# nrlugg/fenix

Hardware: NVIDIA B200
Metric: knn_qps (higher is better)
Workload: dtype f32

## Files before the change

### fenix_b200/csrc/fenix_knn.cu

```cuda
#include <cuda.h>
#include <cuda_runtime.h>
#include <nvtx3/nvToolsExt.h>

#include <dlfcn.h>
#include <unistd.h>

#include <algorithm>
#include <atomic>
#include <chrono>
#include <cmath>
#include <condition_variable>
#include <cstdarg>
#include <cstdio>
#include <cstdlib>
#include <cstring>
#include <memory>
#include <mutex>
#include <new>
#include <string>
#include <thread>
#include <unordered_map>
#include <vector>

#include "../../include/fenix_knn.h"
// ... 115 lines not shown
  fx::TcCorpus tc;
  struct GraphEntry {
    int64_t n_q = 0; int metric = 0, k = 0, precision = 0;
    int state = 0;
    cudaGraphExec_t exec = nullptr;
    void* ptrs[7] = {nullptr, nullptr, nullptr, nullptr, nullptr, nullptr, nullptr};
    uint64_t knob_epoch = 0;
    int path = 0, variant = 0, launches = 0, operand = 0;
  };
  std::vector<GraphEntry> graphs;
  int* d_inv = nullptr; long long* d_cell_off = nullptr;
  std::vector<long long> h_cell_off;
  int64_t n_inv = 0, n_cells = 0;
};

static int bind(fx_ctx* ctx) {
  FX_CUDA(cudaSetDevice(ctx->device));
  return FX_OK;
}

struct HandleState { int users = 0; bool doomed = false; };
static std::mutex g_reg_mu;
static std::condition_variable g_reg_cv;
static std::unordered_map<const fx_corpus*, HandleState> g_live;

struct Lease {
  const fx_corpus* c;
  bool ok = false;
  explicit Lease(const fx_corpus* c_) : c(c_) {
    if (!c) return;
// ... 576 lines not shown
    s.certify = precision == FX_PREC_FP32; s.out_rows = d_out_rows; s.out_dist = d_out_dist;
    s.stream = ctx->stream; s.ev_k0 = ctx->ev_k0; s.ev_k1 = ctx->ev_k1; s.ev_flags = ev_flags; s.dbg = nullptr; s.tau_fixed = nullptr;
    const bool have_i8 = int8_wanted(c, metric, k, precision) && ensure_i8_shadow(c);
    const bool want_bf16 = precision == FX_PREC_BF16 || (precision == FX_PREC_FP32 && !ctx->tc.knobs.fp32_filter_tf32);
    const bool have_shadow = !have_i8 && want_bf16 && ((metric == 1 && ensure_norm_shadow(c)) || ensure_plain_shadow(c));
    const int kind = have_i8 ? 2 : (have_shadow ? 1 : 0);
    if (precision == FX_PREC_BF16 && !have_shadow)
      return fail(FX_ESTATE, "fx_search: FX_PREC_BF16 needs a bf16 shadow (none could be built: FENIX_BF16_SHADOW=0, a tiny shard, or no HBM left)");
    FX_TRY(configure_filter(c, metric, kind, d_mask, &s));
    run->L = fx::tc_prepare(&ctx->tc, s);
    FX_TRY(ctx->d_tc.ensure(run->L.scratch_bytes));
    std::string err;
    int launched = 0, variant = 0;
    if (!fx::tc_search(&ctx->tc, &c->tc, s, run->L, ctx->d_tc.p, &launched, &err, &variant)) return fail(FX_ECUDA, "fx_search: %s", err.c_str());
    run->tc = true; run->path = kind == 0 ? 1 : 2; run->operand = kind;
    c->stats.last_variant = variant;
    ctx->launches += launched; c->stats.kernel_launches += launched;
    if (s.certify) FX_CUDA(cudaMemcpyAsync(ctx->h_word, fx::tc_flag_count(ctx->d_tc.p), sizeof(int), cudaMemcpyDeviceToHost, ctx->stream));
  } else {
    FX_CUDA(cudaEventRecordWithFlags(ctx->ev_k0, ctx->stream, ev_flags));
    FX_TRY(run_exact_scan(c, d_q, int(n_q), nullptr, int(n_q), metric, k, d_mask, d_out_rows, d_out_dist));
    FX_CUDA(cudaEventRecordWithFlags(ctx->ev_k1, ctx->stream, ev_flags));
  }
  if (!spin) FX_CUDA(cudaEventRecordWithFlags(ctx->ev_stop, ctx->stream, ev_flags));
  return FX_OK;
}

static int search_settle(fx_corpus* c, SearchRun* run, bool* changed) {
  fx_ctx* ctx = c->ctx;
  *changed = false;
  if (!run->tc || !run->s.certify || ctx->h_word[0] == 0) return FX_OK;
// ... 176 lines not shown
  ctx->capturing = false;
  cudaGraph_t graph = nullptr;
  const cudaError_t ee = cudaStreamEndCapture(ctx->stream, &graph);
  if (!ok || ee != cudaSuccess || !graph || !run->tc) {
    cudaGetLastError();
    if (graph) cudaGraphDestroy(graph);
    g->state = -1;
    return false;
  }
  cudaGraphExec_t exec = nullptr;
  if (cudaGraphInstantiate(&exec, graph, 0) != cudaSuccess) { cudaGetLastError(); cudaGraphDestroy(graph); g->state = -1; return false; }
  cudaGraphDestroy(graph);
  g->exec = exec; g->state = 1; g->knob_epoch = ctx->knob_epoch;
  const void* now[7] = {ctx->d_q.p, ctx->d_rows.p, ctx->d_dist.p, ctx->d_tc.p, ctx->h_q.p, ctx->h_rows.p, ctx->h_dist.p};
  for (int i = 0; i < 7; ++i) g->ptrs[i] = const_cast<void*>(now[i]);
  g->path = run->path; g->operand = run->operand; g->variant = c->stats.last_variant; g->launches = int(c->stats.kernel_launches - launches0);
  c->stats.kernel_launches = launches0;
  return true;
}

extern "C" int fx_search(fx_corpus* c, const float* queries, int64_t n_q, int32_t metric, int32_t k,
                         int32_t precision, const uint8_t* row_mask, int64_t* out_rows, float* out_dist) {
  FX_LEASE(c, "fx_search");
  NvtxRange nvtx("fenix:search");
  FX_TRY(check_search_args(c, queries, n_q, metric, k, precision, out_rows, out_dist));
  if (n_q == 0) return FX_OK;
  fx_ctx* ctx = c->ctx;
  std::lock_guard<std::mutex> lock(ctx->mu);
  FX_TRY(bind(ctx));
  const size_t q_bytes = size_t(n_q) * c->dim * sizeof(float);
  const size_t r_bytes = size_t(n_q) * k * sizeof(int64_t), d_bytes = size_t(n_q) * k * sizeof(float);
// ... 55 lines not shown
    if (g->state == 1 && !graph_buffers_match(ctx, *g)) {
      cudaGraphExecDestroy(g->exec); g->exec = nullptr; g->state = 0;
    }
    bool launched = false;
    SearchRun run;
    if (g->state >= 0) {
      FX_TRY(ctx->h_q.ensure(q_bytes));
      FX_TRY(ctx->h_rows.ensure(r_bytes));
      FX_TRY(ctx->h_dist.ensure(d_bytes));
    }
    if (g->state == 1) {
      std::memcpy(ctx->h_q.p, queries, q_bytes);
      ctx->h_word[0] = 0;
      FX_CUDA(cudaGraphLaunch(g->exec, ctx->stream));
      run.tc = true; run.path = g->path; run.operand = g->operand; run.n_q = n_q;
      c->stats.last_variant = g->variant;
      ctx->launches += g->launches; c->stats.kernel_launches += g->launches;
      launched = true;
    } else if (g->state == 2) {
      std::memcpy(ctx->h_q.p, queries, q_bytes);
      if (graph_capture(c, g, n_q, metric, k, precision, q_bytes, r_bytes, d_bytes, &run)) {
        ctx->h_word[0] = 0;
        FX_CUDA(cudaGraphLaunch(g->exec, ctx->stream));
        ctx->launches += g->launches; c->stats.kernel_launches += g->launches;
        launched = true;
      }
    } else if (g->state == 0) {
      g->state = 2;
    }
    if (launched) {
      FX_CUDA(cudaStreamSynchronize(ctx->stream));
// ... 607 lines not shown
```

### fenix_b200/csrc/tc_filter.cuh

```cuda
#pragma once
#include <cuda.h>
#include <cuda_bf16.h>
#include <cuda_runtime.h>

#include <cstdlib>
#include <string>

#include "common.cuh"

namespace fx {

constexpr int TC_BM = 128;
constexpr int TC_BN = 256;
constexpr int TC_BK = 32;
constexpr int TC_UMMA_K = 8;
constexpr int TC_STAGES = 4;
constexpr int TC_ACC_STAGES = 2;
constexpr int TC_SPLIT = 2;
#ifndef FENIX_EPI_UNROLL
#define FENIX_EPI_UNROLL 2
#endif
constexpr int TC_EPI_UNROLL = FENIX_EPI_UNROLL;
constexpr int TC_EPI_WARPS = 4 * TC_SPLIT;
constexpr int TC_THREADS = 32 * (4 + TC_EPI_WARPS);
constexpr int TC_EPI_FIRST_WARP = 4;
constexpr int TC_HALF_COLS = TC_BN / TC_SPLIT;
constexpr int TC_SLOTS = TC_SPLIT * TC_BM;
constexpr int TC_CW = 32;
constexpr uint32_t TC_A_BYTES = TC_BM * TC_BK * 4;
constexpr uint32_t TC_B_BYTES = TC_BN * TC_BK * 4;
constexpr uint32_t TC_STAGE_BYTES = TC_A_BYTES + TC_B_BYTES;
constexpr uint32_t TC_NORM_BYTES = TC_BN * 4;
constexpr uint32_t TC_SMEM_BYTES = 1024  + TC_STAGES * TC_STAGE_BYTES +
                                   TC_ACC_STAGES * TC_NORM_BYTES + 512 ;
constexpr int TC2_STAGES = 6;
constexpr uint32_t TC2_B_BYTES = TC_B_BYTES / 2;
constexpr uint32_t TC2_STAGE_BYTES = TC_A_BYTES + TC2_B_BYTES;
constexpr uint32_t TC2_SMEM_BYTES = 1024  + TC2_STAGES * TC2_STAGE_BYTES +
                                    TC_ACC_STAGES * TC_NORM_BYTES + 512 ;
constexpr size_t TC_HDR_BYTES = 256;
constexpr int TC_MAX_WAVES = 4;
constexpr uint32_t ORD_NEG_INF = 0x007fffffu;

constexpr int TC_AUG_COLS = 4;
struct ShadowGeom {
  int n_kb_data;
  int aug_col;
  bool aug_separate;
  int pitch_q;
};
inline ShadowGeom shadow_geom(int dim) {
  ShadowGeom g;
  g.n_kb_data = (dim + 63) / 64;
  const int used = dim - 64 * (g.n_kb_data - 1);
// ... 37 lines not shown
  int pair = -1;
  int errcol = -1;
  int fp32_filter_tf32 = 0;
  int no_refine = 0;
  int no_norm_shadow = 0;
  int debug_bf16 = 0;
  int graph = 1;
  int debug_tiers = 0;
  int direct = 1;
  int direct_mb = 256;
  int direct_spin = 1;
  int direct_qreg = 0;
  int merge_rank_min = 0;
  int debug_direct = 0;
  int int8 = -1;
};
inline bool tc_set_knob(TcKnobs* k, const char* name, const char* value) {
  const std::string n(name ? name : "");
  const TcKnobs d{};
  auto as_int = [&](int dflt) { return value ? std::atoi(value) : dflt; };
  auto as_flag = [&]() { return (value && std::atoi(value) != 0) ? 1 : 0; };
  auto as_dbl = [&]() { return value ? std::atof(value) : 0.0; };
  if (n == "FENIX_TC_KP") k->kp = as_int(d.kp);
  else if (n == "FENIX_TC_FULLK") k->fullk = as_flag();
  else if (n == "FENIX_TC_NO_RQ") k->no_rq = as_flag();
  else if (n == "FENIX_TC_SLICES") k->slices = as_int(d.slices);
  else if (n == "FENIX_TC_MAX_WAVES") k->max_waves = as_int(d.max_waves);
  else if (n == "FENIX_TC_ORDER") k->order = as_int(d.order);
  else if (n == "FENIX_TC_KP_LIST") k->kp_list = as_int(d.kp_list);
  else if (n == "FENIX_TC_PRE_WIDE") k->pre_wide = as_int(d.pre_wide);
// ... 8 lines not shown
  else if (n == "FENIX_TC_PAIR") k->pair = as_int(d.pair);
  else if (n == "FENIX_TC_ERRCOL") k->errcol = as_int(d.errcol);
  else if (n == "FENIX_FP32_FILTER_TF32") k->fp32_filter_tf32 = as_flag();
  else if (n == "FENIX_NO_REFINE") k->no_refine = as_flag();
  else if (n == "FENIX_NO_NORM_SHADOW") k->no_norm_shadow = as_flag();
  else if (n == "FENIX_DEBUG_BF16") k->debug_bf16 = as_flag();
  else if (n == "FENIX_DEBUG_TIERS") k->debug_tiers = as_flag();
  else if (n == "FENIX_GRAPH") k->graph = as_int(d.graph);
  else if (n == "FENIX_DIRECT") k->direct = as_int(d.direct);
  else if (n == "FENIX_DIRECT_MAX_MB") k->direct_mb = as_int(d.direct_mb);
  else if (n == "FENIX_DEBUG_DIRECT") k->debug_direct = as_flag();
  else if (n == "FENIX_DIRECT_SPIN") k->direct_spin = as_int(d.direct_spin);
  else if (n == "FENIX_DIRECT_QREG") k->direct_qreg = as_int(d.direct_qreg);
  else if (n == "FENIX_MERGE_RANK_MIN") k->merge_rank_min = as_int(d.merge_rank_min);
  else if (n == "FENIX_INT8") k->int8 = as_int(d.int8);
  else return false;
  return true;
}
inline void tc_knobs_from_env(TcKnobs* k) {
  static const char* const names[] = {
      "FENIX_TC_KP", "FENIX_TC_FULLK", "FENIX_TC_NO_RQ", "FENIX_TC_SLICES", "FENIX_TC_MAX_WAVES", "FENIX_TC_ORDER", "FENIX_TC_KP_LIST",
      "FENIX_TC_PRE_WIDE", "FENIX_TC_PRE", "FENIX_TC_PRE_SMALL", "FENIX_TC_PRE_SAFETY", "FENIX_TC_PRE_M", "FENIX_TC_PF", "FENIX_RQ_STAGES",
      "FENIX_FIN_THREADS", "FENIX_TC_WARM", "FENIX_TC_PAIR", "FENIX_TC_ERRCOL", "FENIX_FP32_FILTER_TF32", "FENIX_NO_REFINE",
      "FENIX_NO_NORM_SHADOW", "FENIX_DEBUG_BF16", "FENIX_DEBUG_TIERS", "FENIX_GRAPH", "FENIX_DIRECT", "FENIX_DIRECT_MAX_MB", "FENIX_DEBUG_DIRECT", "FENIX_DIRECT_SPIN", "FENIX_DIRECT_QREG", "FENIX_MERGE_RANK_MIN", "FENIX_INT8"};
  for (const char* name : names) {
    if (const char* v = std::getenv(name)) tc_set_knob(k, name, v);
  }
}

struct TcState {
  int sm_count = 0;
  void* encode = nullptr;
  TcKnobs knobs;
};
struct TcCorpus {
  CUtensorMap map_x;
  CUtensorMap map_xb;
  CUtensorMap map_xn;
  CUtensorMap map_xb_h, map_xn_h;
// ... 529 lines not shown
    uint32_t v_ord = (p.cap == 1024) ? warp_select_compact<32>(b, c_src, p.kp, new_cnt)
                                     : warp_select_compact<16>(b, c_src, p.kp, new_cnt);
    if (int(lane) == src) {
      wn = uint32_t(new_cnt);
      tau = fmaxf(tau, ord2f(v_ord));
      atomicMax(p.tau_g + q, v_ord);
      wn_trig = epi_trigger(p, active, tau);
    }
  }
}

template <int METRIC, int KIND, int MODE, int PAIR>
__global__ void __launch_bounds__(TC_THREADS, 1)
knn_tc_filter_kernel(const __grid_constant__ CUtensorMap map_q, const __grid_constant__ CUtensorMap map_x, TcParams p) {
  static_assert(!PAIR || KIND >= 1, "CTA pairs stream a shadow");
  constexpr int STAGES = PAIR ? TC2_STAGES : TC_STAGES;
  constexpr uint32_t B_BYTES = PAIR ? TC2_B_BYTES : TC_B_BYTES;
  constexpr uint32_t STAGE_BYTES = TC_A_BYTES + B_BYTES;
  extern __shared__ unsigned char smem_raw[];
  unsigned char* smem = smem_raw + ((1024u - (smem_u32(smem_raw) & 1023u)) & 1023u);
  unsigned char* tiles = smem;
  float* norm_smem = reinterpret_cast<float*>(smem + STAGES * STAGE_BYTES);
  uint64_t* bars = reinterpret_cast<uint64_t*>(smem + STAGES * STAGE_BYTES + TC_ACC_STAGES * TC_NORM_BYTES);
  uint64_t* full_bar = bars;
  uint64_t* empty_bar = bars + STAGES;
  uint64_t* tmem_full = bars + 2 * STAGES;
  uint64_t* tmem_empty = tmem_full + TC_ACC_STAGES;
  uint64_t* norm_full = tmem_empty + TC_ACC_STAGES;
  uint64_t* norm_empty = norm_full + TC_ACC_STAGES;
  uint32_t* tmem_ptr = reinterpret_cast<uint32_t*>(norm_empty + TC_ACC_STAGES);

  const int warp = threadIdx.x >> 5;
  const uint32_t lane = lane_id();
  const uint32_t rank = PAIR ? cluster_ctarank() : 0u;
  const int cid = PAIR ? int(blockIdx.x >> 1) : int(blockIdx.x);
  const int n_workers = PAIR ? int(gridDim.x >> 1) : int(gridDim.x);

  if (warp == 0 && lane == 0) {
    prefetch_tmap(&map_q);
    prefetch_tmap(&map_x);
    for (int i = 0; i < STAGES; ++i) { mbar_init(&full_bar[i], 1); mbar_init(&empty_bar[i], 1); }
    for (int i = 0; i < TC_ACC_STAGES; ++i) {
      mbar_init(&tmem_full[i], 1);
      mbar_init(&tmem_empty[i], PAIR ? 2 * TC_EPI_WARPS : TC_EPI_WARPS);
      mbar_init(&norm_full[i], 1);
      mbar_init(&norm_empty[i], TC_EPI_WARPS);
    }
    fence_barrier_init();
  }
  if (warp == 2) { if (PAIR) tmem_alloc_pair(tmem_ptr, 512); else tmem_alloc(tmem_ptr, 512); }
  tc_fence_before();
  __syncthreads();
  if (PAIR) cluster_sync_all();
  tc_fence_after();
  const uint32_t tmem_base = *tmem_ptr;

  const int n_qp = (p.n_qt + 1) >> 1;
  const int n_units = PAIR ? p.n_slices * n_qp : p.n_slices * p.n_qt;
  const int n_rows_i = int(p.n_rows);
  auto decode = [&](int u, int& qt, int& slice, int& cu) {
    if (PAIR) { const int qp = u % n_qp; slice = u / n_qp; qt = 2 * qp + int(rank); cu = slice * (2 * n_qp) + qt; }
    else { qt = p.qt_major ? u / p.n_slices : u % p.n_qt; slice = p.qt_major ? u % p.n_slices : u / p.n_qt; cu = u; }
  };

  if (warp == 0) {
    if (lane == 0) {
      int stage = 0; uint32_t phase = 0;
      int acc = 0; uint32_t acc_phase = 0;
      const uint32_t full_leader = PAIR ? mapa_u32(smem_u32(full_bar), 0) : 0u;
      for (int u = cid; u < n_units; u += n_workers) {
        int qt, slice, cu; decode(u, qt, slice, cu);
        const int t0 = slice * p.tiles_per_slice, t1 = min(p.n_vtiles, t0 + p.tiles_per_slice);
        for (int tv = t0; tv < t1; ++tv) {
          const int t = tv * p.tile_stride;
          if (METRIC != 2) {
            mbar_wait_backoff(PAIR ? &norm_empty[acc] : &tmem_empty[acc], acc_phase ^ 1, p.sleep_ns);
            mbar_expect_tx(&norm_full[acc], TC_NORM_BYTES);
            const float* src = (METRIC == 0 ? p.hx : p.rx) + size_t(t) * TC_BN;
            bulk_load_1d(norm_smem + acc * TC_BN, src, TC_NORM_BYTES, &norm_full[acc]);
          }
          for (int kb = 0; kb < p.n_kblocks; ++kb) {
            mbar_wait_backoff(&empty_bar[stage], phase ^ 1, p.sleep_ns);
            unsigned char* a_dst = tiles + stage * STAGE_BYTES;
            constexpr int kElemsPerBlock = KIND == 0 ? TC_BK : (KIND == 1 ? 2 * TC_BK : 4 * TC_BK);
            const int line = kb < p.n_kb_data ? (t * p.n_kb_data + kb) * TC_BN : p.aug_line0 + t * TC_BN;
            if (PAIR) {
              if (rank == 0) mbar_expect_tx(&full_bar[stage], 2 * STAGE_BYTES);
              const uint32_t bar = full_leader + uint32_t(stage) * 8u;
              tma_load_2d_pair(&map_q, bar, a_dst, kb * kElemsPerBlock, qt * TC_BM);
              tma_load_2d_pair(&map_x, bar, a_dst + TC_A_BYTES, 0, line + int(rank) * (TC_BN / 2));
            } else {
              mbar_expect_tx(&full_bar[stage], STAGE_BYTES);
              tma_load_2d(&map_q, &full_bar[stage], a_dst, kb * kElemsPerBlock, qt * TC_BM);
              if (KIND == 0) tma_load_2d(&map_x, &full_bar[stage], a_dst + TC_A_BYTES, kb * kElemsPerBlock, t * TC_BN);
              else {
                tma_load_2d(&map_x, &full_bar[stage], a_dst + TC_A_BYTES, 0, line);
#ifndef FENIX_NO_PFCODE
                if (p.pf_tiles > 0 && tv + p.pf_tiles < t1) {
                  const int tp = (tv + p.pf_tiles) * p.tile_stride;
                  const int64_t linep = kb < p.n_kb_data ? (int64_t(tp) * p.n_kb_data + kb) * TC_BN : int64_t(p.aug_line0) + int64_t(tp) * TC_BN;
                  prefetch_l2(p.xb + linep * 128, TC_B_BYTES);
                }
#endif
              }
            }
            if (++stage == STAGES) { stage = 0; phase ^= 1; }
          }
          if (++acc == TC_ACC_STAGES) { acc = 0; acc_phase ^= 1; }
        }
      }
    }
  } else if (warp == 1 && rank == 0) {
    {
      constexpr uint32_t idesc = KIND == 0 ? make_idesc_tf32(TC_BM, TC_BN)
                                           : KIND == 1 ? make_idesc_bf16(PAIR ? 2 * TC_BM : TC_BM, TC_BN)
                                                       : make_idesc_i8(PAIR ? 2 * TC_BM : TC_BM, TC_BN);
      const uint32_t tmem_u = __shfl_sync(0xffffffffu, tmem_base, 0);
      const uint64_t desc0 = make_smem_desc(0);
      const uint32_t tiles_lo = smem_u32(tiles) >> 4;
      const int n_kb = p.n_kblocks, n_kb_data = p.n_kb_data, nk_last = p.nk_last;
      int stage = 0; uint32_t phase = 0;
      int acc = 0; uint32_t acc_phase = 0;
      for (int u = cid; u < n_units; u += n_workers) {
        int qt, slice, cu; decode(u, qt, slice, cu);
        const int t0 = slice * p.tiles_per_slice, t1 = min(p.n_vtiles, t0 + p.tiles_per_slice);
        for (int t = t0; t < t1; ++t) {
          mbar_wait_backoff(&tmem_empty[acc], acc_phase ^ 1, p.sleep_ns >> 1);
          const uint32_t d_tmem = tmem_u + uint32_t(acc * TC_BN);
          for (int kb = 0; kb < n_kb; ++kb) {
            mbar_wait(&full_bar[stage], phase);
            tc_fence_after();
            const uint64_t a_desc = desc0 | uint64_t(tiles_lo + uint32_t(stage) * (STAGE_BYTES >> 4));
            const uint64_t b_desc = a_desc + (TC_A_BYTES >> 4);
            const int nk = kb < n_kb_data - 1 ? TC_BK / TC_UMMA_K : (kb == n_kb_data - 1 ? nk_last : 1);
            if (elect_one()) {
              if (PAIR && KIND == 2) {
                umma_i8_pair(d_tmem, a_desc, b_desc, idesc, kb != 0 ? 1u : 0u);
                if (nk > 1) umma_i8_pair(d_tmem, a_desc + 2, b_desc + 2, idesc, 1u);
                if (nk > 2) umma_i8_pair(d_tmem, a_desc + 4, b_desc + 4, idesc, 1u);
                if (nk > 3) umma_i8_pair(d_tmem, a_desc + 6, b_desc + 6, idesc, 1u);
                umma_commit_pair(&empty_bar[stage]);
                if (kb == n_kb - 1) umma_commit_pair(&tmem_full[acc]);
              } else if (PAIR) {
                umma_bf16_pair(d_tmem, a_desc, b_desc, idesc, kb != 0 ? 1u : 0u);
                if (nk > 1) umma_bf16_pair(d_tmem, a_desc + 2, b_desc + 2, idesc, 1u);
                if (nk > 2) umma_bf16_pair(d_tmem, a_desc + 4, b_desc + 4, idesc, 1u);
                if (nk > 3) umma_bf16_pair(d_tmem, a_desc + 6, b_desc + 6, idesc, 1u);
                umma_commit_pair(&empty_bar[stage]);
// ... 8 lines not shown
                  umma_bf16(d_tmem, a_desc, b_desc, idesc, kb != 0 ? 1u : 0u);
                  if (nk > 1) umma_bf16(d_tmem, a_desc + 2, b_desc + 2, idesc, 1u);
                  if (nk > 2) umma_bf16(d_tmem, a_desc + 4, b_desc + 4, idesc, 1u);
                  if (nk > 3) umma_bf16(d_tmem, a_desc + 6, b_desc + 6, idesc, 1u);
                } else {
                  umma_i8(d_tmem, a_desc, b_desc, idesc, kb != 0 ? 1u : 0u);
                  if (nk > 1) umma_i8(d_tmem, a_desc + 2, b_desc + 2, idesc, 1u);
                  if (nk > 2) umma_i8(d_tmem, a_desc + 4, b_desc + 4, idesc, 1u);
                  if (nk > 3) umma_i8(d_tmem, a_desc + 6, b_desc + 6, idesc, 1u);
                }
                umma_commit(&empty_bar[stage]);
                if (kb == n_kb - 1) umma_commit(&tmem_full[acc]);
              }
            }
            __syncwarp();
            if (++stage == STAGES) { stage = 0; phase ^= 1; }
          }
          if (++acc == TC_ACC_STAGES) { acc = 0; acc_phase ^= 1; }
        }
      }
    }
  } else if (warp >= TC_EPI_FIRST_WARP) {
    const int e = warp - TC_EPI_FIRST_WARP;
    const int lane_grp = warp & 3;
    const int half = e >> 2;
    const int row_in_tile = lane_grp * 32 + int(lane);
    const int slot = half * TC_BM + row_in_tile;
    const uint32_t t_lane = tmem_base + (uint32_t(lane_grp * 32) << 16) + uint32_t(half * TC_HALF_COLS);
    const uint32_t tmem_empty_leader = PAIR ? mapa_u32(smem_u32(tmem_empty), 0) : 0u;
    int acc = 0; uint32_t acc_phase = 0;

    for (int u = cid; u < n_units; u += n_workers) {
      int qt, slice, cu; decode(u, qt, slice, cu);
// ... 20 lines not shown
        float2 ts = make_float2(1.f, 0.f);
        if (KIND == 2) ts = __ldg(p.i8_tile + t);
        mbar_wait(&tmem_full[acc], acc_phase);
        if (METRIC != 2) mbar_wait(&norm_full[acc], acc_phase);
        tc_fence_after();
        const int col0 = t * TC_BN + half * TC_HALF_COLS;
        const int ncols = min(TC_HALF_COLS, n_rows_i - col0);
        const float* nrm = norm_smem + acc * TC_BN + half * TC_HALF_COLS;
        float* dbg_row = nullptr;
        if (MODE == 1) { if (u == 0 && tv == t0) dbg_row = p.dbg + (int(lane) * 4 + lane_grp) * TC_BN + half * TC_HALF_COLS; }
        float* pre_out = nullptr;
        if (MODE == 2) { if (active) pre_out = p.pre_max + size_t(q) * p.pre_pitch + (tv * TC_SPLIT + half); }
        if (KIND == 2) {
          const double ss = double(ts.x) * double(qs.x);
          const double ae = fma(double(qs.y), double(ts.y), double(qs.z)) + 0x1p-48;
          epi_tile_i8<METRIC, MODE, PAIR>(t_lane + uint32_t(acc * TC_BN), any_active ? ncols : 0, nrm, col0, tau,
                                          i8_threshold(tau, ss, ae), 1.0 / ss, ae, buf, wn, &tmem_empty[acc],
                                          tmem_empty_leader + uint32_t(acc) * 8u, &norm_empty[acc], lane, dbg_row, pre_out);
        } else {
          epi_tile<METRIC, MODE, PAIR>(t_lane + uint32_t(acc * TC_BN), any_active ? ncols : 0, nrm, col0, tau, buf, wn,
                                       &tmem_empty[acc], tmem_empty_leader + uint32_t(acc) * 8u, &norm_empty[acc], lane, dbg_row, pre_out);
        }
        if (++acc == TC_ACC_STAGES) { acc = 0; acc_phase ^= 1; }
        if (MODE != 2) epi_tighten(p, active, q, buf, wn, wn_trig, tau, lane);
      }

      if (MODE != 2) p.wcnt[size_t(cu) * TC_SLOTS + slot] = active ? int(wn) : 0;
    }
  }

  tc_fence_before();
  __syncthreads();
  if (PAIR) cluster_sync_all();
  if (warp == 2) {
    tc_fence_after();
    if (PAIR) tmem_dealloc_pair(tmem_base, 512); else tmem_dealloc(tmem_base, 512);
// ... 766 lines not shown
    if (a == cudaSuccess) a = cudaFuncSetAttribute(kernel, cudaFuncAttributeMaxDynamicSharedMemorySize, int(bytes));
  };
  attr(knn_tc_filter_kernel<0, 0, 0, 0>, TC_SMEM_BYTES); attr(knn_tc_filter_kernel<1, 0, 0, 0>, TC_SMEM_BYTES);
  attr(knn_tc_filter_kernel<2, 0, 0, 0>, TC_SMEM_BYTES); attr(knn_tc_filter_kernel<0, 1, 0, 0>, TC_SMEM_BYTES);
  attr(knn_tc_filter_kernel<1, 1, 0, 0>, TC_SMEM_BYTES); attr(knn_tc_filter_kernel<2, 1, 0, 0>, TC_SMEM_BYTES);
  attr(knn_tc_filter_kernel<0, 1, 2, 0>, TC_SMEM_BYTES); attr(knn_tc_filter_kernel<1, 1, 2, 0>, TC_SMEM_BYTES);
  attr(knn_tc_filter_kernel<2, 1, 2, 0>, TC_SMEM_BYTES);
  attr(knn_tc_filter_kernel<0, 1, 0, 1>, TC2_SMEM_BYTES); attr(knn_tc_filter_kernel<1, 1, 0, 1>, TC2_SMEM_BYTES);
  attr(knn_tc_filter_kernel<2, 1, 0, 1>, TC2_SMEM_BYTES);
  attr(knn_tc_filter_kernel<0, 1, 2, 1>, TC2_SMEM_BYTES); attr(knn_tc_filter_kernel<1, 1, 2, 1>, TC2_SMEM_BYTES);
  attr(knn_tc_filter_kernel<2, 1, 2, 1>, TC2_SMEM_BYTES);
  attr(knn_tc_filter_kernel<0, 2, 0, 0>, TC_SMEM_BYTES); attr(knn_tc_filter_kernel<2, 2, 0, 0>, TC_SMEM_BYTES);
  attr(knn_tc_filter_kernel<2, 2, 2, 0>, TC_SMEM_BYTES);
  attr(knn_tc_filter_kernel<0, 2, 0, 1>, TC2_SMEM_BYTES); attr(knn_tc_filter_kernel<2, 2, 0, 1>, TC2_SMEM_BYTES);
  attr(knn_tc_filter_kernel<2, 2, 2, 1>, TC2_SMEM_BYTES);
  if (a == cudaSuccess) a = cudaFuncSetAttribute(knn_rq_filter_kernel<0, 0>, cudaFuncAttributeMaxDynamicSharedMemorySize, RQ_SMEM_MAX);
  if (a == cudaSuccess) a = cudaFuncSetAttribute(knn_rq_filter_kernel<0, 2>, cudaFuncAttributeMaxDynamicSharedMemorySize, RQ_SMEM_MAX);
  if (a == cudaSuccess) a = cudaFuncSetAttribute(knn_rq_filter_kernel<2, 2>, cudaFuncAttributeMaxDynamicSharedMemorySize, RQ_SMEM_MAX);
  if (a == cudaSuccess) a = cudaFuncSetAttribute(knn_rq_filter_kernel<2, 0>, cudaFuncAttributeMaxDynamicSharedMemorySize, RQ_SMEM_MAX);
  if (a == cudaSuccess) a = cudaFuncSetAttribute(knn_tc_finish_kernel, cudaFuncAttributeMaxDynamicSharedMemorySize, 64 * 1024);
  if (a != cudaSuccess) { *err = std::string("cudaFuncSetAttribute(tc kernels) failed: ") + cudaGetErrorString(a); return false; }
  return true;
}

inline bool tc_bind_shadow(const TcState* st, CUtensorMap* map, CUtensorMap* map_half, const void* Xb, int64_t n_rows,
                           int blocks_per_tile, std::string* err, int esize = 2) {
  const uint64_t lines = uint64_t((n_rows + TC_BN - 1) / TC_BN) * uint64_t(blocks_per_tile) * TC_BN;
  if (lines >= (uint64_t(1) << 31)) { *err = "shard too large for a tiled shadow (32-bit TMA coordinates)"; return false; }
  const uint32_t line = 128 / esize;
  if (!tc_encode_2d(st, map_half, Xb, line, lines, line, line, TC_BN / 2, err, esize)) return false;
// ... 26 lines not shown
  (void)n_q;
  if (!st->encode || !tc->ok) return false;
  if (dim > 8192) return false;
  if (k > 320) return false;
  if (n_rows < 4096 || n_rows < 8 * int64_t(k)) return false;
  if (n_rows > int64_t(0x7fffff00)) return false;
  return true;
}

struct TcPlan {
  int n_qt, n_tiles, n_slices, tiles_per_slice, grid, units, kp, cap, n_kblocks, n_kb_data, nk_last, aug_line0, aug_col;
  int n_vtiles, tile_stride;
  int qt_major;
  int rq;
  int pair;
  int n_qt_lists;
  int n_qp;
  int kp_list;
  int kb_bf16;
  size_t off_qp, off_qb, off_tau, off_flags, off_qerr, off_wcnt, off_wbuf, off_pre, total;
  int n_rec, pre_pitch;
};

inline TcPlan tc_plan(const TcState* st, const TcSearch& s) {
  TcPlan pl{};
  pl.n_qt = (s.n_q + TC_BM - 1) / TC_BM;
  pl.n_tiles = int((s.n_rows + TC_BN - 1) / TC_BN);
  pl.kp = s.tau_fixed ? 1024 : tc_kp(s.k, s.certify, s.kind);
  const bool pre = s.sample_stride > 1;
  if (pre) pl.kp = 32;
// ... 10 lines not shown
    pl.nk_last = (s.dim - I8_KB * (pl.n_kb_data - 1) + 31) / 32;
    pl.n_kblocks = pl.n_kb_data;
  } else {
    const ShadowGeom g = shadow_geom(s.dim);
    pl.n_kb_data = g.n_kb_data;
    const int used = s.dim - 64 * (g.n_kb_data - 1) + ((s.aug && !g.aug_separate) ? TC_AUG_COLS : 0);
    pl.nk_last = (used + 15) / 16;
    pl.n_kblocks = g.n_kb_data + ((s.aug && g.aug_separate) ? 1 : 0);
    pl.aug_line0 = pl.n_tiles * g.n_kb_data * TC_BN;
    pl.aug_col = g.aug_col;
  }
  if (kn.fullk) pl.nk_last = TC_BK / TC_UMMA_K;
  pl.kb_bf16 = s.kind == 2 ? (s.dim + 63) / 64 : pl.n_kblocks;
  pl.rq = (s.kind == 1 && pl.n_kblocks <= RQ_MAX_KB && pl.n_qt >= 2 && s.epi != 1 && s.dbg == nullptr && !kn.no_rq) ? 1 : 0;
  pl.n_qp = (pl.n_qt + 1) / 2;
  pl.pair = (!pl.rq && s.kind >= 1 && pl.n_qt >= 2 && s.dbg == nullptr && (kn.pair == 1 || (kn.pair < 0 && pl.kb_bf16 >= 7))) ? 1 : 0;
  pl.n_qt_lists = pl.pair ? 2 * pl.n_qp : pl.n_qt;
  const int n_tiles_full = pl.rq ? int((s.n_rows + RQ_BN - 1) / RQ_BN) : pl.n_tiles;
  pl.tile_stride = pre ? s.sample_stride : 1;
  const int n_tiles_u = (n_tiles_full + pl.tile_stride - 1) / pl.tile_stride;
  pl.n_vtiles = n_tiles_u;
  const int n_qu = (pl.rq || pl.pair) ? pl.n_qp : pl.n_qt;
  const int sms = pl.pair ? st->sm_count / 2 : st->sm_count;
  const int min_tiles = pre ? 4 : std::max(4, (8 * pl.kp + TC_BN - 1) / TC_BN) * (pl.rq ? 2 : 1);
  const int max_waves = kn.max_waves > 0 ? kn.max_waves : TC_MAX_WAVES;
  const int s_cap = std::max(1, (max_waves * sms) / n_qu);
  const int s_max = std::max(1, std::min(n_tiles_u / min_tiles, s_cap));
  double best = -1.0; int best_s = 1;
  for (int sl = 1; sl <= s_max; ++sl) {
    int tps = (n_tiles_u + sl - 1) / sl;
    int eff_s = (n_tiles_u + tps - 1) / tps;
// ... 160 lines not shown
    le = cudaLaunchKernelEx(&cfg, kernel, map_q, map_b, p);
  };
  const bool dbg = s.dbg != nullptr;
  if (pl.rq) {
    const CUtensorMap& map_h = s.shadow == 1 ? tc->map_xn_h : tc->map_xb_h;
    p.rq_stages = rq_stages(pl.n_kblocks);
    if (st->knobs.rq_stages >= 2 && st->knobs.rq_stages <= p.rq_stages) p.rq_stages = st->knobs.rq_stages;
    const uint32_t rq_smem = rq_smem_bytes(pl.n_kblocks);
    if (pre) {
      if (epi == 0) launch(knn_rq_filter_kernel<0, 2>, map_h, rq_smem, 1);
      else launch(knn_rq_filter_kernel<2, 2>, map_h, rq_smem, 1);
    } else {
      if (epi == 0) launch(knn_rq_filter_kernel<0, 0>, map_h, rq_smem, 1);
      else launch(knn_rq_filter_kernel<2, 0>, map_h, rq_smem, 1);
    }
  } else if (pl.pair && s.kind == 2) {
    if (epi == 0) launch(knn_tc_filter_kernel<0, 2, 0, 1>, tc->map_x8_h, TC2_SMEM_BYTES, 2);
    else if (pre) launch(knn_tc_filter_kernel<2, 2, 2, 1>, tc->map_x8_h, TC2_SMEM_BYTES, 2);
    else launch(knn_tc_filter_kernel<2, 2, 0, 1>, tc->map_x8_h, TC2_SMEM_BYTES, 2);
  } else if (s.kind == 2) {
    if (dbg) {
      cudaFuncSetAttribute(knn_tc_filter_kernel<2, 2, 1, 0>, cudaFuncAttributeMaxDynamicSharedMemorySize, TC_SMEM_BYTES);
      launch(knn_tc_filter_kernel<2, 2, 1, 0>, tc->map_x8, TC_SMEM_BYTES, 1);
    } else if (epi == 0) launch(knn_tc_filter_kernel<0, 2, 0, 0>, tc->map_x8, TC_SMEM_BYTES, 1);
    else if (pre) launch(knn_tc_filter_kernel<2, 2, 2, 0>, tc->map_x8, TC_SMEM_BYTES, 1);
    else launch(knn_tc_filter_kernel<2, 2, 0, 0>, tc->map_x8, TC_SMEM_BYTES, 1);
  } else if (pl.pair) {
    const CUtensorMap& map_h = s.shadow == 1 ? tc->map_xn_h : tc->map_xb_h;
#define FX_TC2_CASE(E)                                                              \
  if (epi == E) {                                                                   \
// ... 73 lines not shown
  float* qerr = reinterpret_cast<float*>(base + pl.off_qerr);
  const bool aug = s.kind == 1 && s.aug != 0;
  *launched = 3;
  if (aug) {
    knn_qerr_kernel<<<(s.n_q + 3) / 4, 128, 0, s.stream>>>(s.Q, s.n_q, s.dim, s.c_pair, qerr);
    *launched += 1;
  }
  knn_prep_kernel<<<std::max(prep_blocks, 1), 256, 0, s.stream>>>(s.Q, s.n_q, n_rows_p, s.dim, s.pitch, qp, tau_g, flags, qb, s.pitch_b, s.tau_fixed,
                                                                  (!s.tau_fixed && st->knobs.warm) ? 1 : 0,
                                                                  aug ? pl.aug_col : 0, reinterpret_cast<int*>(base), s.aug, qerr);
  if (s.kind == 2) {
    knn_qprep_i8_kernel<<<(n_rows_p + 7) / 8, 256, 0, s.stream>>>(s.Q, s.n_q, n_rows_p, s.dim, s.pitch_b,
                                                                 reinterpret_cast<int8_t*>(base + pl.off_qb), reinterpret_cast<float4*>(qerr));
    *launched += 1;
  }
  if (variant) *variant = (pl.rq ? 1 : 0) | (L.with_pre ? 2 : 0) | (pl.pair ? 4 : 0);
  if (L.with_pre) {
    if (!tc_run_pass(st, tc, L.pre, L.ppl, scratch, map_q, err)) return false;
    *launched += 2;
  }
  return tc_run_pass(st, tc, s, pl, scratch, map_q, err);
}

}
```

### fenix_b200/knn.py

```python
from __future__ import annotations

import ctypes
import os
import threading
import weakref
from dataclasses import dataclass
from typing import Optional

import numpy as np

__all__ = [
    "FenixKnnError", "Context", "Corpus", "Comm", "Group", "Stats", "METRICS", "metric_code",
    "PREC_FP32", "PREC_TF32", "PREC_BF16", "PREC_EXACT_SCAN", "load_library", "library_path", "COMM_ID_BYTES",
]

_HERE = os.path.dirname(os.path.abspath(__file__))
_LIB_NAME = "libfenix_knn.so"
COMM_ID_BYTES = 128
ABI_VERSION = 4

FX_OK = 0
FX_EINVAL, FX_ECUDA, FX_ENOMEM, FX_ESTATE, FX_EUNSUP = -1, -2, -3, -4, -5
PREC_FP32, PREC_TF32, PREC_BF16, PREC_EXACT_SCAN = 0, 1, 2, 3

METRICS = {"l2": 0, "euclidean": 0, "cosine": 1, "dot": 2, "inner_product": 2}

ABI_SYMBOLS = (
    "fx_init", "fx_shutdown", "fx_corpus_create", "fx_corpus_append", "fx_corpus_append_device",
    "fx_corpus_finalize", "fx_corpus_destroy", "fx_search", "fx_search_device", "fx_distances",
    "fx_merge_topk", "fx_get_stats", "fx_debug_scores", "fx_last_error", "fx_abi_version", "fx_set_option",
    "fx_comm_unique_id", "fx_comm_init_rank", "fx_comm_destroy", "fx_search_sharded", "fx_search_sharded_device",
    "fx_group_create", "fx_group_size", "fx_group_ctx", "fx_group_search", "fx_group_destroy",
    "fx_corpus_set_cells", "fx_search_cells",
)
# ... 8 lines not shown

def metric_code(metric: str) -> int:
    try:
        return METRICS[metric]
    except KeyError:
        raise ValueError(f"unknown metric {metric!r}") from None


class _FxStats(ctypes.Structure):
    _fields_ = [
        ("n_rows", ctypes.c_int64), ("dim", ctypes.c_int32), ("pitch", ctypes.c_int32),
        ("device_bytes", ctypes.c_int64), ("searches", ctypes.c_int64), ("queries", ctypes.c_int64),
        ("fallback_queries", ctypes.c_int64), ("refined_queries", ctypes.c_int64), ("kernel_launches", ctypes.c_int64),
        ("last_search_ms", ctypes.c_double), ("last_main_kernel_ms", ctypes.c_double),
        ("last_path", ctypes.c_int32), ("last_variant", ctypes.c_int32), ("last_exchange_ms", ctypes.c_double),
        ("last_operand", ctypes.c_int32),
    ]


@dataclass(frozen=True)
class Stats:
    n_rows: int
    dim: int
    pitch: int
    device_bytes: int
    searches: int
    queries: int
    fallback_queries: int
    refined_queries: int
    kernel_launches: int
    last_search_ms: float
    last_main_kernel_ms: float
    last_path: int
    last_variant: int = 0
    last_exchange_ms: float = 0.0
    last_operand: int = 0


_lib_lock = threading.Lock()
_lib: Optional[ctypes.CDLL] = None


def library_path() -> str:
    return os.environ.get("FENIX_KNN_LIB", os.path.join(_HERE, _LIB_NAME))


def load_library() -> ctypes.CDLL:
    global _lib
    with _lib_lock:
        if _lib is not None:
            return _lib
# ... 347 lines not shown
```

### include/fenix_knn.h

```cpp
#ifndef FENIX_KNN_H_
#define FENIX_KNN_H_

#include <stddef.h>
#include <stdint.h>

#ifdef __cplusplus
extern "C" {
#endif

#define FX_ABI_VERSION 4

#define FX_OK 0
#define FX_EINVAL (-1)
#define FX_ECUDA (-2)
#define FX_ENOMEM (-3)
#define FX_ESTATE (-4)
#define FX_EUNSUP (-5)

#define FX_METRIC_L2 0
#define FX_METRIC_COSINE 1
#define FX_METRIC_IP 2

#define FX_PREC_FP32 0
#define FX_PREC_TF32 1
#define FX_PREC_BF16 2
// ... 10 lines not shown
  int64_t n_rows;
  int32_t dim;
  int32_t pitch;
  int64_t device_bytes;
  int64_t searches;
  int64_t queries;
  int64_t fallback_queries;
  int64_t refined_queries;
  int64_t kernel_launches;
  double last_search_ms;
  double last_main_kernel_ms;
  int32_t last_path;
  int32_t last_variant;
  double last_exchange_ms;
  int32_t last_operand;
} fx_stats;


int fx_init(int device, fx_ctx** out);
int fx_shutdown(fx_ctx* ctx);

int fx_corpus_create(fx_ctx* ctx, int64_t capacity_rows, int32_t dim, int32_t dtype,
                     int64_t row_base, fx_corpus** out);

int fx_corpus_append(fx_corpus* c, const void* host_rows, int64_t n_rows);

int fx_corpus_append_device(fx_corpus* c, const void* device_rows, int64_t n_rows);

int fx_corpus_finalize(fx_corpus* c);

// ... 51 lines not shown
```

Measured before the change: 142,800.

## Keep int8 query tile resident in shared memory for paired TC filter

Adds a resident-query variant of the paired int8 tensor-core filter kernel. The whole query tile (all k-blocks) is loaded once per work unit into shared memory, and only corpus tiles stream through a deeper stage ring sized to the remaining shared memory. This removes the repeated TMA reload of the query A-tile for every corpus tile and k-block, cutting shared-memory fill traffic. The cost is less room for pipeline stages and a new A-buffer barrier handshake that serialises query tile switches between units. It is enabled by default only for int8 operands on large corpora (at least 4M rows) when pairing is already chosen.

```diff
diff --git a/fenix_b200/csrc/fenix_knn.cu b/fenix_b200/csrc/fenix_knn.cu
--- a/fenix_b200/csrc/fenix_knn.cu
+++ b/fenix_b200/csrc/fenix_knn.cu
@@ -153,6 +153,11 @@
   int64_t n_inv = 0, n_cells = 0;
 };
 
+static void set_variant(fx_corpus* c, int variant) {
+  c->stats.last_variant = variant & 7;
+  c->stats.last_resident_queries = (variant >> 3) & 1;
+}
+
 static int bind(fx_ctx* ctx) {
   FX_CUDA(cudaSetDevice(ctx->device));
   return FX_OK;
@@ -759,7 +764,7 @@
     int launched = 0, variant = 0;
     if (!fx::tc_search(&ctx->tc, &c->tc, s, run->L, ctx->d_tc.p, &launched, &err, &variant)) return fail(FX_ECUDA, "fx_search: %s", err.c_str());
     run->tc = true; run->path = kind == 0 ? 1 : 2; run->operand = kind;
-    c->stats.last_variant = variant;
+    set_variant(c, variant);
     ctx->launches += launched; c->stats.kernel_launches += launched;
     if (s.certify) FX_CUDA(cudaMemcpyAsync(ctx->h_word, fx::tc_flag_count(ctx->d_tc.p), sizeof(int), cudaMemcpyDeviceToHost, ctx->stream));
   } else {
@@ -966,7 +971,7 @@
   g->exec = exec; g->state = 1; g->knob_epoch = ctx->knob_epoch;
   const void* now[7] = {ctx->d_q.p, ctx->d_rows.p, ctx->d_dist.p, ctx->d_tc.p, ctx->h_q.p, ctx->h_rows.p, ctx->h_dist.p};
   for (int i = 0; i < 7; ++i) g->ptrs[i] = const_cast<void*>(now[i]);
-  g->path = run->path; g->operand = run->operand; g->variant = c->stats.last_variant; g->launches = int(c->stats.kernel_launches - launches0);
+  g->path = run->path; g->operand = run->operand; g->variant = c->stats.last_variant | (c->stats.last_resident_queries << 3); g->launches = int(c->stats.kernel_launches - launches0);
   c->stats.kernel_launches = launches0;
   return true;
 }
@@ -1052,7 +1057,7 @@
       ctx->h_word[0] = 0;
       FX_CUDA(cudaGraphLaunch(g->exec, ctx->stream));
       run.tc = true; run.path = g->path; run.operand = g->operand; run.n_q = n_q;
-      c->stats.last_variant = g->variant;
+      set_variant(c, g->variant);
       ctx->launches += g->launches; c->stats.kernel_launches += g->launches;
       launched = true;
     } else if (g->state == 2) {
diff --git a/fenix_b200/csrc/tc_filter.cuh b/fenix_b200/csrc/tc_filter.cuh
--- a/fenix_b200/csrc/tc_filter.cuh
+++ b/fenix_b200/csrc/tc_filter.cuh
@@ -38,6 +38,19 @@
 constexpr uint32_t TC2_STAGE_BYTES = TC_A_BYTES + TC2_B_BYTES;
 constexpr uint32_t TC2_SMEM_BYTES = 1024  + TC2_STAGES * TC2_STAGE_BYTES +
                                     TC_ACC_STAGES * TC_NORM_BYTES + 512 ;
+constexpr int TC3_MAX_STAGES = 12;
+constexpr uint32_t TC3_SMEM_MAX = 227 * 1024;
+constexpr uint32_t TC3_FIXED_BYTES = 1024  + TC_ACC_STAGES * TC_NORM_BYTES + 512 ;
+constexpr int TC3_MIN_STAGES = 4;
+inline int tc3_stages(int n_kblocks) {
+  const int s = (int(TC3_SMEM_MAX) - int(TC3_FIXED_BYTES) - n_kblocks * int(TC_A_BYTES)) / int(TC2_B_BYTES);
+  return s < TC3_MAX_STAGES ? s : TC3_MAX_STAGES;
+}
+inline uint32_t tc3_smem_bytes(int n_kblocks) {
+  return TC3_FIXED_BYTES + uint32_t(n_kblocks) * TC_A_BYTES + uint32_t(tc3_stages(n_kblocks)) * TC2_B_BYTES;
+}
+static_assert(TC3_FIXED_BYTES + 6 * TC_A_BYTES + 7 * TC2_B_BYTES <= TC3_SMEM_MAX, "D = 768 (6 int8 k-blocks): 7 corpus stages");
+static_assert(TC3_FIXED_BYTES + 9 * TC_A_BYTES + TC3_MIN_STAGES * TC2_B_BYTES <= TC3_SMEM_MAX, "D <= 1152: 4 corpus stages");
 constexpr size_t TC_HDR_BYTES = 256;
 constexpr int TC_MAX_WAVES = 4;
 constexpr uint32_t ORD_NEG_INF = 0x007fffffu;
@@ -105,6 +118,7 @@
   int merge_rank_min = 0;
   int debug_direct = 0;
   int int8 = -1;
+  int resident = -1;
 };
 inline bool tc_set_knob(TcKnobs* k, const char* name, const char* value) {
   const std::string n(name ? name : "");
@@ -143,6 +157,7 @@
   else if (n == "FENIX_DIRECT_QREG") k->direct_qreg = as_int(d.direct_qreg);
   else if (n == "FENIX_MERGE_RANK_MIN") k->merge_rank_min = as_int(d.merge_rank_min);
   else if (n == "FENIX_INT8") k->int8 = as_int(d.int8);
+  else if (n == "FENIX_TC_RESIDENT") k->resident = as_int(d.resident);
   else return false;
   return true;
 }
@@ -151,7 +166,7 @@
       "FENIX_TC_KP", "FENIX_TC_FULLK", "FENIX_TC_NO_RQ", "FENIX_TC_SLICES", "FENIX_TC_MAX_WAVES", "FENIX_TC_ORDER", "FENIX_TC_KP_LIST",
       "FENIX_TC_PRE_WIDE", "FENIX_TC_PRE", "FENIX_TC_PRE_SMALL", "FENIX_TC_PRE_SAFETY", "FENIX_TC_PRE_M", "FENIX_TC_PF", "FENIX_RQ_STAGES",
       "FENIX_FIN_THREADS", "FENIX_TC_WARM", "FENIX_TC_PAIR", "FENIX_TC_ERRCOL", "FENIX_FP32_FILTER_TF32", "FENIX_NO_REFINE",
-      "FENIX_NO_NORM_SHADOW", "FENIX_DEBUG_BF16", "FENIX_DEBUG_TIERS", "FENIX_GRAPH", "FENIX_DIRECT", "FENIX_DIRECT_MAX_MB", "FENIX_DEBUG_DIRECT", "FENIX_DIRECT_SPIN", "FENIX_DIRECT_QREG", "FENIX_MERGE_RANK_MIN", "FENIX_INT8"};
+      "FENIX_NO_NORM_SHADOW", "FENIX_DEBUG_BF16", "FENIX_DEBUG_TIERS", "FENIX_GRAPH", "FENIX_DIRECT", "FENIX_DIRECT_MAX_MB", "FENIX_DEBUG_DIRECT", "FENIX_DIRECT_SPIN", "FENIX_DIRECT_QREG", "FENIX_MERGE_RANK_MIN", "FENIX_INT8", "FENIX_TC_RESIDENT"};
   for (const char* name : names) {
     if (const char* v = std::getenv(name)) tc_set_knob(k, name, v);
   }
@@ -711,21 +726,27 @@
 __global__ void __launch_bounds__(TC_THREADS, 1)
 knn_tc_filter_kernel(const __grid_constant__ CUtensorMap map_q, const __grid_constant__ CUtensorMap map_x, TcParams p) {
   static_assert(!PAIR || KIND >= 1, "CTA pairs stream a shadow");
-  constexpr int STAGES = PAIR ? TC2_STAGES : TC_STAGES;
+  constexpr bool RES = PAIR == 2;
+  static_assert(!RES || KIND == 2, "resident query tiles: int8 shadow");
+  constexpr int STAGES = RES ? TC3_MAX_STAGES : (PAIR ? TC2_STAGES : TC_STAGES);
   constexpr uint32_t B_BYTES = PAIR ? TC2_B_BYTES : TC_B_BYTES;
-  constexpr uint32_t STAGE_BYTES = TC_A_BYTES + B_BYTES;
+  constexpr uint32_t STAGE_BYTES = (RES ? 0u : TC_A_BYTES) + B_BYTES;
+  const int n_stages = RES ? p.rq_stages : STAGES;
   extern __shared__ unsigned char smem_raw[];
   unsigned char* smem = smem_raw + ((1024u - (smem_u32(smem_raw) & 1023u)) & 1023u);
-  unsigned char* tiles = smem;
-  float* norm_smem = reinterpret_cast<float*>(smem + STAGES * STAGE_BYTES);
-  uint64_t* bars = reinterpret_cast<uint64_t*>(smem + STAGES * STAGE_BYTES + TC_ACC_STAGES * TC_NORM_BYTES);
+  unsigned char* a_res = smem;
+  unsigned char* tiles = RES ? smem + p.n_kblocks * TC_A_BYTES : smem;
+  float* norm_smem = reinterpret_cast<float*>(tiles + n_stages * STAGE_BYTES);
+  uint64_t* bars = reinterpret_cast<uint64_t*>(tiles + n_stages * STAGE_BYTES + TC_ACC_STAGES * TC_NORM_BYTES);
   uint64_t* full_bar = bars;
   uint64_t* empty_bar = bars + STAGES;
   uint64_t* tmem_full = bars + 2 * STAGES;
   uint64_t* tmem_empty = tmem_full + TC_ACC_STAGES;
   uint64_t* norm_full = tmem_empty + TC_ACC_STAGES;
   uint64_t* norm_empty = norm_full + TC_ACC_STAGES;
-  uint32_t* tmem_ptr = reinterpret_cast<uint32_t*>(norm_empty + TC_ACC_STAGES);
+  uint64_t* a_full = norm_empty + TC_ACC_STAGES;
+  uint64_t* a_empty = a_full + 1;
+  uint32_t* tmem_ptr = reinterpret_cast<uint32_t*>(a_full + (RES ? 2 : 0));
 
   const int warp = threadIdx.x >> 5;
   const uint32_t lane = lane_id();
@@ -736,13 +757,14 @@
   if (warp == 0 && lane == 0) {
     prefetch_tmap(&map_q);
     prefetch_tmap(&map_x);
-    for (int i = 0; i < STAGES; ++i) { mbar_init(&full_bar[i], 1); mbar_init(&empty_bar[i], 1); }
+    for (int i = 0; i < n_stages; ++i) { mbar_init(&full_bar[i], 1); mbar_init(&empty_bar[i], 1); }
     for (int i = 0; i < TC_ACC_STAGES; ++i) {
       mbar_init(&tmem_full[i], 1);
       mbar_init(&tmem_empty[i], PAIR ? 2 * TC_EPI_WARPS : TC_EPI_WARPS);
       mbar_init(&norm_full[i], 1);
       mbar_init(&norm_empty[i], TC_EPI_WARPS);
     }
+    if (RES) { mbar_init(a_full, 1); mbar_init(a_empty, 1); }
     fence_barrier_init();
   }
   if (warp == 2) { if (PAIR) tmem_alloc_pair(tmem_ptr, 512); else tmem_alloc(tmem_ptr, 512); }
@@ -765,9 +787,19 @@
       int stage = 0; uint32_t phase = 0;
       int acc = 0; uint32_t acc_phase = 0;
       const uint32_t full_leader = PAIR ? mapa_u32(smem_u32(full_bar), 0) : 0u;
+      constexpr int kElemsPerBlock = KIND == 0 ? TC_BK : (KIND == 1 ? 2 * TC_BK : 4 * TC_BK);
+      uint32_t a_phase = 0;
       for (int u = cid; u < n_units; u += n_workers) {
         int qt, slice, cu; decode(u, qt, slice, cu);
         const int t0 = slice * p.tiles_per_slice, t1 = min(p.n_vtiles, t0 + p.tiles_per_slice);
+        if (RES) {
+          mbar_wait_backoff(a_empty, a_phase ^ 1, p.sleep_ns);
+          if (rank == 0) mbar_expect_tx(a_full, 2u * uint32_t(p.n_kblocks) * TC_A_BYTES);
+          const uint32_t a_bar = mapa_u32(smem_u32(a_full), 0);
+          for (int kb = 0; kb < p.n_kblocks; ++kb)
+            tma_load_2d_pair(&map_q, a_bar, a_res + kb * TC_A_BYTES, kb * kElemsPerBlock, qt * TC_BM);
+          a_phase ^= 1;
+        }
         for (int tv = t0; tv < t1; ++tv) {
           const int t = tv * p.tile_stride;
           if (METRIC != 2) {
@@ -779,9 +811,11 @@
           for (int kb = 0; kb < p.n_kblocks; ++kb) {
             mbar_wait_backoff(&empty_bar[stage], phase ^ 1, p.sleep_ns);
             unsigned char* a_dst = tiles + stage * STAGE_BYTES;
-            constexpr int kElemsPerBlock = KIND == 0 ? TC_BK : (KIND == 1 ? 2 * TC_BK : 4 * TC_BK);
             const int line = kb < p.n_kb_data ? (t * p.n_kb_data + kb) * TC_BN : p.aug_line0 + t * TC_BN;
-            if (PAIR) {
+            if (RES) {
+              if (rank == 0) mbar_expect_tx(&full_bar[stage], 2 * STAGE_BYTES);
+              tma_load_2d_pair(&map_x, full_leader + uint32_t(stage) * 8u, a_dst, 0, line + int(rank) * (TC_BN / 2));
+            } else if (PAIR) {
               if (rank == 0) mbar_expect_tx(&full_bar[stage], 2 * STAGE_BYTES);
               const uint32_t bar = full_leader + uint32_t(stage) * 8u;
               tma_load_2d_pair(&map_q, bar, a_dst, kb * kElemsPerBlock, qt * TC_BM);
@@ -801,7 +835,7 @@
 #endif
               }
             }
-            if (++stage == STAGES) { stage = 0; phase ^= 1; }
+            if (++stage == n_stages) { stage = 0; phase ^= 1; }
           }
           if (++acc == TC_ACC_STAGES) { acc = 0; acc_phase ^= 1; }
         }
@@ -815,20 +849,25 @@
       const uint32_t tmem_u = __shfl_sync(0xffffffffu, tmem_base, 0);
       const uint64_t desc0 = make_smem_desc(0);
       const uint32_t tiles_lo = smem_u32(tiles) >> 4;
+      const uint32_t a_lo = smem_u32(a_res) >> 4;
       const int n_kb = p.n_kblocks, n_kb_data = p.n_kb_data, nk_last = p.nk_last;
       int stage = 0; uint32_t phase = 0;
       int acc = 0; uint32_t acc_phase = 0;
+      uint32_t a_phase = 0;
       for (int u = cid; u < n_units; u += n_workers) {
         int qt, slice, cu; decode(u, qt, slice, cu);
         const int t0 = slice * p.tiles_per_slice, t1 = min(p.n_vtiles, t0 + p.tiles_per_slice);
+        if (RES) { mbar_wait(a_full, a_phase); a_phase ^= 1; }
         for (int t = t0; t < t1; ++t) {
           mbar_wait_backoff(&tmem_empty[acc], acc_phase ^ 1, p.sleep_ns >> 1);
           const uint32_t d_tmem = tmem_u + uint32_t(acc * TC_BN);
           for (int kb = 0; kb < n_kb; ++kb) {
             mbar_wait(&full_bar[stage], phase);
             tc_fence_after();
-            const uint64_t a_desc = desc0 | uint64_t(tiles_lo + uint32_t(stage) * (STAGE_BYTES >> 4));
-            const uint64_t b_desc = a_desc + (TC_A_BYTES >> 4);
+            const uint64_t a_desc = RES ? desc0 | uint64_t(a_lo + uint32_t(kb) * (TC_A_BYTES >> 4))
+                                        : desc0 | uint64_t(tiles_lo + uint32_t(stage) * (STAGE_BYTES >> 4));
+            const uint64_t b_desc = RES ? desc0 | uint64_t(tiles_lo + uint32_t(stage) * (STAGE_BYTES >> 4))
+                                        : a_desc + (TC_A_BYTES >> 4);
             const int nk = kb < n_kb_data - 1 ? TC_BK / TC_UMMA_K : (kb == n_kb_data - 1 ? nk_last : 1);
             if (elect_one()) {
               if (PAIR && KIND == 2) {
@@ -867,9 +906,13 @@
               }
             }
             __syncwarp();
-            if (++stage == STAGES) { stage = 0; phase ^= 1; }
+            if (++stage == n_stages) { stage = 0; phase ^= 1; }
           }
           if (++acc == TC_ACC_STAGES) { acc = 0; acc_phase ^= 1; }
+        }
+        if (RES && u + n_workers < n_units) {
+          if (elect_one()) umma_commit_pair(a_empty);
+          __syncwarp();
         }
       }
     }
@@ -920,12 +963,12 @@
         if (KIND == 2) {
           const double ss = double(ts.x) * double(qs.x);
           const double ae = fma(double(qs.y), double(ts.y), double(qs.z)) + 0x1p-48;
-          epi_tile_i8<METRIC, MODE, PAIR>(t_lane + uint32_t(acc * TC_BN), any_active ? ncols : 0, nrm, col0, tau,
-                                          i8_threshold(tau, ss, ae), 1.0 / ss, ae, buf, wn, &tmem_empty[acc],
-                                          tmem_empty_leader + uint32_t(acc) * 8u, &norm_empty[acc], lane, dbg_row, pre_out);
+          epi_tile_i8<METRIC, MODE, (PAIR != 0)>(t_lane + uint32_t(acc * TC_BN), any_active ? ncols : 0, nrm, col0, tau,
+                                                    i8_threshold(tau, ss, ae), 1.0 / ss, ae, buf, wn, &tmem_empty[acc],
+                                                    tmem_empty_leader + uint32_t(acc) * 8u, &norm_empty[acc], lane, dbg_row, pre_out);
         } else {
-          epi_tile<METRIC, MODE, PAIR>(t_lane + uint32_t(acc * TC_BN), any_active ? ncols : 0, nrm, col0, tau, buf, wn,
-                                       &tmem_empty[acc], tmem_empty_leader + uint32_t(acc) * 8u, &norm_empty[acc], lane, dbg_row, pre_out);
+          epi_tile<METRIC, MODE, (PAIR != 0)>(t_lane + uint32_t(acc * TC_BN), any_active ? ncols : 0, nrm, col0, tau, buf, wn,
+                                                 &tmem_empty[acc], tmem_empty_leader + uint32_t(acc) * 8u, &norm_empty[acc], lane, dbg_row, pre_out);
         }
         if (++acc == TC_ACC_STAGES) { acc = 0; acc_phase ^= 1; }
         if (MODE != 2) epi_tighten(p, active, q, buf, wn, wn_trig, tau, lane);
@@ -1722,6 +1765,8 @@
   attr(knn_tc_filter_kernel<2, 2, 2, 0>, TC_SMEM_BYTES);
   attr(knn_tc_filter_kernel<0, 2, 0, 1>, TC2_SMEM_BYTES); attr(knn_tc_filter_kernel<2, 2, 0, 1>, TC2_SMEM_BYTES);
   attr(knn_tc_filter_kernel<2, 2, 2, 1>, TC2_SMEM_BYTES);
+  attr(knn_tc_filter_kernel<0, 2, 0, 2>, TC3_SMEM_MAX); attr(knn_tc_filter_kernel<2, 2, 0, 2>, TC3_SMEM_MAX);
+  attr(knn_tc_filter_kernel<2, 2, 2, 2>, TC3_SMEM_MAX);
   if (a == cudaSuccess) a = cudaFuncSetAttribute(knn_rq_filter_kernel<0, 0>, cudaFuncAttributeMaxDynamicSharedMemorySize, RQ_SMEM_MAX);
   if (a == cudaSuccess) a = cudaFuncSetAttribute(knn_rq_filter_kernel<0, 2>, cudaFuncAttributeMaxDynamicSharedMemorySize, RQ_SMEM_MAX);
   if (a == cudaSuccess) a = cudaFuncSetAttribute(knn_rq_filter_kernel<2, 2>, cudaFuncAttributeMaxDynamicSharedMemorySize, RQ_SMEM_MAX);
@@ -1778,6 +1823,7 @@
   int qt_major;
   int rq;
   int pair;
+  int resident;
   int n_qt_lists;
   int n_qp;
   int kp_list;
@@ -1818,7 +1864,12 @@
   pl.kb_bf16 = s.kind == 2 ? (s.dim + 63) / 64 : pl.n_kblocks;
   pl.rq = (s.kind == 1 && pl.n_kblocks <= RQ_MAX_KB && pl.n_qt >= 2 && s.epi != 1 && s.dbg == nullptr && !kn.no_rq) ? 1 : 0;
   pl.n_qp = (pl.n_qt + 1) / 2;
-  pl.pair = (!pl.rq && s.kind >= 1 && pl.n_qt >= 2 && s.dbg == nullptr && (kn.pair == 1 || (kn.pair < 0 && pl.kb_bf16 >= 7))) ? 1 : 0;
+  const bool pair_ok = !pl.rq && s.kind >= 1 && pl.n_qt >= 2 && s.dbg == nullptr;
+  pl.pair = (pair_ok && (kn.pair == 1 || (kn.pair < 0 && pl.kb_bf16 >= 7))) ? 1 : 0;
+  constexpr int64_t TC3_MIN_ROWS = int64_t(1) << 22;
+  const bool res_fits = s.kind == 2 && tc3_stages(pl.n_kblocks) >= TC3_MIN_STAGES;
+  pl.resident = (pair_ok && res_fits && (kn.resident == 1 || (kn.resident < 0 && pl.pair && s.n_rows >= TC3_MIN_ROWS))) ? 1 : 0;
+  if (pl.resident) pl.pair = 1;
   pl.n_qt_lists = pl.pair ? 2 * pl.n_qp : pl.n_qt;
   const int n_tiles_full = pl.rq ? int((s.n_rows + RQ_BN - 1) / RQ_BN) : pl.n_tiles;
   pl.tile_stride = pre ? s.sample_stride : 1;
@@ -2009,6 +2060,12 @@
       if (epi == 0) launch(knn_rq_filter_kernel<0, 0>, map_h, rq_smem, 1);
       else launch(knn_rq_filter_kernel<2, 0>, map_h, rq_smem, 1);
     }
+  } else if (pl.resident) {
+    p.rq_stages = tc3_stages(pl.n_kblocks);
+    const uint32_t smem = tc3_smem_bytes(pl.n_kblocks);
+    if (epi == 0) launch(knn_tc_filter_kernel<0, 2, 0, 2>, tc->map_x8_h, smem, 2);
+    else if (pre) launch(knn_tc_filter_kernel<2, 2, 2, 2>, tc->map_x8_h, smem, 2);
+    else launch(knn_tc_filter_kernel<2, 2, 0, 2>, tc->map_x8_h, smem, 2);
   } else if (pl.pair && s.kind == 2) {
     if (epi == 0) launch(knn_tc_filter_kernel<0, 2, 0, 1>, tc->map_x8_h, TC2_SMEM_BYTES, 2);
     else if (pre) launch(knn_tc_filter_kernel<2, 2, 2, 1>, tc->map_x8_h, TC2_SMEM_BYTES, 2);
@@ -2112,7 +2169,7 @@
                                                                  reinterpret_cast<int8_t*>(base + pl.off_qb), reinterpret_cast<float4*>(qerr));
     *launched += 1;
   }
-  if (variant) *variant = (pl.rq ? 1 : 0) | (L.with_pre ? 2 : 0) | (pl.pair ? 4 : 0);
+  if (variant) *variant = (pl.rq ? 1 : 0) | (L.with_pre ? 2 : 0) | (pl.pair ? 4 : 0) | (pl.resident ? 8 : 0);
   if (L.with_pre) {
     if (!tc_run_pass(st, tc, L.pre, L.ppl, scratch, map_q, err)) return false;
     *launched += 2;
diff --git a/fenix_b200/knn.py b/fenix_b200/knn.py
--- a/fenix_b200/knn.py
+++ b/fenix_b200/knn.py
@@ -17,7 +17,7 @@
 _HERE = os.path.dirname(os.path.abspath(__file__))
 _LIB_NAME = "libfenix_knn.so"
 COMM_ID_BYTES = 128
-ABI_VERSION = 4
+ABI_VERSION = 5
 
 FX_OK = 0
 FX_EINVAL, FX_ECUDA, FX_ENOMEM, FX_ESTATE, FX_EUNSUP = -1, -2, -3, -4, -5
@@ -56,7 +56,7 @@
         ("fallback_queries", ctypes.c_int64), ("refined_queries", ctypes.c_int64), ("kernel_launches", ctypes.c_int64),
         ("last_search_ms", ctypes.c_double), ("last_main_kernel_ms", ctypes.c_double),
         ("last_path", ctypes.c_int32), ("last_variant", ctypes.c_int32), ("last_exchange_ms", ctypes.c_double),
-        ("last_operand", ctypes.c_int32),
+        ("last_operand", ctypes.c_int32), ("last_resident_queries", ctypes.c_int32),
     ]
 
 
@@ -77,6 +77,7 @@
     last_variant: int = 0
     last_exchange_ms: float = 0.0
     last_operand: int = 0
+    last_resident_queries: int = 0
 
 
 _lib_lock = threading.Lock()
diff --git a/include/fenix_knn.h b/include/fenix_knn.h
--- a/include/fenix_knn.h
+++ b/include/fenix_knn.h
@@ -8,7 +8,7 @@
 extern "C" {
 #endif
 
-#define FX_ABI_VERSION 4
+#define FX_ABI_VERSION 5
 
 #define FX_OK 0
 #define FX_EINVAL (-1)
@@ -49,6 +49,7 @@
   int32_t last_variant;
   double last_exchange_ms;
   int32_t last_operand;
+  int32_t last_resident_queries;
 } fx_stats;
 
 
```

After: 150,400, median of 6. 5.3% higher.
